# HKUST-Aerial-Robotics/VINS-Mono

Measured on AMD Instinct MI355X. Metric: sliding-window BA solves/sec (Estimator::optimization: 8-iteration dogleg solve + marginalization), higher is better.
Workload: dtype f64; 1 GPU; batch of 256 independent EuRoC-shape windows per step and GPU (K=11 frames, ~150 landmarks, 10 IMU factors, ~600 projection factors, 75-dim marginalization prior, max 8 iterations, MARGIN_OLD marginalization); windows resident in HBM; consecutive steps are issued to 16 HIP streams (independent batches in flight); windows_per_gpu=256, batches_in_flight=16, parallelism=independent batches x1 (no collectives)

## Files before the change

include/vinsgpu.h:

```cpp
#ifndef VINSGPU_H
#define VINSGPU_H
#include <stddef.h>
#include <stdint.h>
#ifdef __cplusplus
extern "C" {
#endif

#define VG_ABI_VERSION 12
#define VG_MAX_ITERS 32

typedef enum {
    VG_OK = 0,
    VG_ERR_BAD_ARG = -1,
    VG_ERR_HIP = -2,
    VG_ERR_UNSUPPORTED = -3,
    VG_ERR_NUMERIC = -4,
    VG_ERR_NO_DEVICE = -5
} vg_status;

typedef struct vg_handle vg_handle;

int vg_abi_version(void);
int vg_create(vg_handle** out);
typedef struct vg_config {
// ... 300 lines not shown
       VG_BA_KERNEL_BIG_SCHUR, VG_BA_KERNEL_BIG_SOLVE, VG_BA_KERNEL_BIG_STEP, VG_BA_KERNEL_COUNT };
int vg_ba_batch_run_profiled(vg_handle* h, float* ms, int* n);
int vg_ba_batch_flops_by_kernel(vg_handle* h, double* flops);
int vg_ba_batch_info(vg_handle* h, double* flops_per_run, double* bytes_in, double* bytes_out, int* lds_bytes);
int vg_ba_batch_flops(vg_handle* h, double* solve_flops, double* marg_flops);

typedef int (*vg_allreduce_fn)(void* user, double* device_buf, size_t count, void* stream);
int vg_ba_set_allreduce(vg_handle* h, vg_allreduce_fn fn, void* user);
int vg_ba_set_large_window(vg_handle* h, int force);

#define VG_RCCL_ID_BYTES 128
int vg_rccl_unique_id(char* id128);
int vg_ba_rccl_init(vg_handle* h, int nranks, int rank, const char* id128);
int vg_ba_rccl_finalize(vg_handle* h);

enum { VG_LAUNCH_DIRECT = 0, VG_LAUNCH_GRAPH = 1 };
#ifndef VG_LAUNCH_DEFAULT
#define VG_LAUNCH_DEFAULT VG_LAUNCH_DIRECT
#endif
int vg_ba_set_launch_mode(vg_handle* h, int mode);
int vg_ba_launch_stats(vg_handle* h, int* mode, long long* graph_launches, long long* graph_captures);
int vg_ba_set_fused_min_windows(vg_handle* h, int min_windows);
int vg_ba_batch_is_fused(vg_handle* h);

int vg_ba_reserve(vg_handle* h, int max_landmarks, int max_factors, int max_obs, int max_prior_n);

typedef struct {
    int n_features;
    const int* feature_id;
    const int* start_frame;
    const int* n_obs;
    const int* solve_flag;
    const double* depth;
    const double* obs;
} vg_ba_tracks;

typedef struct {
    int max_features;
    int max_new_obs;
    int max_landmarks;
    int max_factors;
    double init_depth;
    double min_parallax;
} vg_ba_seq_config;

typedef struct {
// ... 446 lines not shown
```

vins-mono_amd/ba.py:

```python
import time
import ctypes as C
import numpy as np

from . import lib

VG_MAX_ITERS = 32
VG_MARGIN_OLD, VG_MARGIN_SECOND_NEW, VG_MARGIN_NONE = 0, 1, 2
VG_MARG_SQRT, VG_MARG_EIGEN = 0, 1
MARGPATH_STAGE1 = (None, 'direct', 'block_lds', 'block_glb', 'vh_eig', 'jacobi_lds', 'jacobi_glb') + (None,) * 9
MARGPATH_CERT = (None, 'passed', 'failed', None)
MARGPATH_SCHUR = (None, 'lds', 'glb', None)
MARGPATH_STAGE2 = (None, 'sqrt', 'sqrt_glb', 'vh_eig', 'jacobi_lds', 'jacobi_glb') + (None,) * 10
VG_IMU_INFO_FACTOR, VG_IMU_INFO_REFERENCE = 0, 1
VG_OK = 0
VG_ABI_VERSION = 12
VG_LAUNCH_DIRECT, VG_LAUNCH_GRAPH = 0, 1
VG_LAUNCH_DEFAULT = VG_LAUNCH_DIRECT
VG_PRIOR_RESIDENT = -1
_pd = C.POINTER(C.c_double)
_pi = C.POINTER(C.c_int)


class ImuPreint(C.Structure):
    _fields_ = [("sum_dt", C.c_double), ("delta_p", C.c_double * 3), ("delta_q", C.c_double * 4),
                ("delta_v", C.c_double * 3), ("linearized_ba", C.c_double * 3), ("linearized_bg", C.c_double * 3),
                ("jacobian", C.c_double * 225), ("covariance", C.c_double * 225), ("valid", C.c_int), ("_pad", C.c_int)]


class Problem(C.Structure):
    _fields_ = [("K", C.c_int), ("L", C.c_int), ("n_obs", C.c_int),
                ("pose", _pd), ("speedbias", _pd), ("ex_pose", _pd), ("td", C.c_double), ("inv_depth", _pd),
# ... 292 lines not shown
        L.vg_create.argtypes = [C.POINTER(C.c_void_p)]
        L.vg_destroy.argtypes = [C.c_void_p]
        L.vg_sync.argtypes = [C.c_void_p]
        L.vg_last_error.argtypes = [C.c_void_p]
        L.vg_last_error.restype = C.c_char_p
        L.vg_timer_start.argtypes = [C.c_void_p]
        L.vg_timer_stop.argtypes = [C.c_void_p, C.POINTER(C.c_float)]
        L.vg_ba_batch_upload.argtypes = [C.c_void_p, C.c_int, C.POINTER(C.POINTER(Problem)), _pi]
        L.vg_ba_batch_run_async.argtypes = [C.c_void_p]
        L.vg_ba_batch_download.argtypes = [C.c_void_p, C.c_int, C.POINTER(C.POINTER(State)), C.POINTER(Summary),
                                           C.POINTER(C.POINTER(Prior))]
        L.vg_ba_batch_download_state.argtypes = [C.c_void_p, C.c_int, C.POINTER(C.POINTER(State)), C.POINTER(Summary)]
        L.vg_ba_batch_download_prior.argtypes = [C.c_void_p, C.c_int, C.POINTER(C.POINTER(Prior))]
        L.vg_ba_batch_run_timed.argtypes = [C.c_void_p, C.POINTER(C.c_float), C.POINTER(C.c_float)]
        L.vg_ba_batch_run_profiled.argtypes = [C.c_void_p, C.POINTER(C.c_float), _pi]
        L.vg_ba_batch_flops_by_kernel.argtypes = [C.c_void_p, _pd]
        L.vg_ba_batch_info.argtypes = [C.c_void_p, _pd, _pd, _pd, _pi]
        L.vg_ba_batch_flops.argtypes = [C.c_void_p, _pd, _pd]
        L.vg_ba_eval_factors.argtypes = [C.c_void_p, C.POINTER(Problem), _pd, _pd, _pd, _pd, _pd]
        L.vg_ba_set_large_window.argtypes = [C.c_void_p, C.c_int]
        L.vg_ba_set_marg_mode.argtypes = [C.c_void_p, C.c_int]
        L.vg_ba_set_launch_mode.argtypes = [C.c_void_p, C.c_int]
        L.vg_ba_set_fused_min_windows.argtypes = [C.c_void_p, C.c_int]
        L.vg_host_register.argtypes = [C.c_void_p, C.c_void_p, C.c_size_t]
        L.vg_host_unregister.argtypes = [C.c_void_p, C.c_void_p]
        L.vg_ba_launch_stats.argtypes = [C.c_void_p, _pi, C.POINTER(C.c_longlong), C.POINTER(C.c_longlong)]
        if hasattr(L, 'vg_ba_rccl_init'):
            L.vg_ba_rccl_init.argtypes = [C.c_void_p, C.c_int, C.c_int, C.c_char_p]
            L.vg_ba_rccl_finalize.argtypes = [C.c_void_p]
        L.vg_ba_set_allreduce.argtypes = [C.c_void_p, ALLREDUCE_FN, C.c_void_p]
        L.vg_ba_reduce_layout.argtypes = [C.c_void_p, C.POINTER(C.c_size_t), C.POINTER(C.c_size_t)]
        L.vg_triangulate.argtypes = [C.c_void_p, C.c_int, _pd, _pd, _pd, _pd, C.c_int, _pi, _pi, _pi, _pd, C.c_double, _pd]
        L.vg_imu_preintegrate.argtypes = [C.c_void_p, C.c_int, _pi, _pd, _pd, _pd, _pd, C.POINTER(ImuPreint)]
        L.vg_ba_reserve.argtypes = [C.c_void_p, C.c_int, C.c_int, C.c_int, C.c_int]
        L.vg_ba_seq_begin.argtypes = [C.c_void_p, C.c_int, C.POINTER(SeqConfig), C.POINTER(C.POINTER(Problem)), C.POINTER(C.POINTER(Tracks))]
        L.vg_ba_seq_step_async.argtypes = [C.c_void_p, C.c_int, C.POINTER(C.POINTER(Frame))]
        L.vg_ba_seq_info.argtypes = [C.c_void_p, C.c_int, _pi]
        L.vg_ba_seq_get_tracks.argtypes = [C.c_void_p, C.c_int, C.c_int, _pi, _pi, _pi, _pi, _pi, _pd, _pd]
        L.vg_ba_seq_end.argtypes = [C.c_void_p]
        L.vg_ba_seq_export.argtypes = [C.c_void_p, C.c_int, _pd, _pd, _pd, _pd, C.POINTER(ImuPreint), C.POINTER(Prior)]
        L.vg_ba_seq_import.argtypes = [C.c_void_p, C.c_int, C.POINTER(Problem), C.POINTER(Tracks)]
        if hasattr(L, "vg_ba_seq_imu_begin"):
            L.vg_ba_seq_imu_begin.argtypes = [C.c_void_p, C.c_int, C.POINTER(SeqImuConfig), _pd]
            L.vg_ba_seq_step_imu_async.argtypes = [C.c_void_p, C.c_int, C.POINTER(C.POINTER(FrameImu))]
            L.vg_ba_seq_imu_get.argtypes = [C.c_void_p, C.c_int, _pd, _pd, _pd]
            L.vg_ba_seq_imu_set.argtypes = [C.c_void_p, C.c_int, _pd]
# ... 70 lines not shown
            n = len(self._packed)
            arr = (C.POINTER(Problem) * n)(*[C.pointer(p.struct) for p in self._packed])
        mf = np.ascontiguousarray(margin_flags if margin_flags is not None else [VG_MARGIN_NONE] * n, dtype=np.int32)
        self._margin = mf
        t0 = time.perf_counter()
        self._chk(self.lib.vg_ba_batch_upload(self.h, n, arr, _ip(mf)), "vg_ba_batch_upload")
        self.last_upload_call_ms = (time.perf_counter() - t0) * 1e3

    def ba_run_async(self):
        self._chk(self.lib.vg_ba_batch_run_async(self.h), "vg_ba_batch_run_async")

    def ba_set_launch_mode(self, mode):
        self._chk(self.lib.vg_ba_set_launch_mode(self.h, int(mode)), "vg_ba_set_launch_mode")

    def host_register(self, arr):
        self._chk(self.lib.vg_host_register(self.h, C.c_void_p(arr.ctypes.data), C.c_size_t(arr.nbytes)), "vg_host_register")

    def host_unregister(self, arr):
        self._chk(self.lib.vg_host_unregister(self.h, C.c_void_p(arr.ctypes.data)), "vg_host_unregister")

    def ba_set_fused_min_windows(self, n):
        self._chk(self.lib.vg_ba_set_fused_min_windows(self.h, int(n)), "vg_ba_set_fused_min_windows")

    def probe_clocks(self):
        out = (C.c_double * 4)()
        self.lib.vg_probe_clocks.argtypes = [C.c_void_p, C.POINTER(C.c_double)]
        self._chk(self.lib.vg_probe_clocks(self.h, out), "vg_probe_clocks")
        return {"lone_wave": {"ns_per_dependent_fma": out[0], "clock64_ticks_per_us": out[1]},
                "all_cus_loaded": {"ns_per_dependent_fma": out[2], "clock64_ticks_per_us": out[3]}}

    def ba_launch_stats(self):
        mode, nl, ncap = C.c_int(), C.c_longlong(), C.c_longlong()
        self._chk(self.lib.vg_ba_launch_stats(self.h, C.byref(mode), C.byref(nl), C.byref(ncap)), "vg_ba_launch_stats")
        return {"mode": "graph" if mode.value == VG_LAUNCH_GRAPH else "direct", "graph_launches": nl.value, "graph_captures": ncap.value}

    def ba_set_marg_mode(self, mode):
        self._chk(self.lib.vg_ba_set_marg_mode(self.h, int(mode)), "vg_ba_set_marg_mode")

    def ba_marg_info(self, window=0):
        self.lib.vg_ba_batch_marg_info.argtypes = [C.c_void_p, C.c_int, C.POINTER(C.c_int)]
        out = (C.c_int * 8)()
        self._chk(self.lib.vg_ba_batch_marg_info(self.h, int(window), out), "vg_ba_batch_marg_info")
        w = int(out[6])
        return dict(valid=int(out[0]), n=int(out[1]), m=int(out[2]), nblocks=int(out[3]), eig1=int(out[4]), eig2=int(out[5]), word=w,
                    stage1=MARGPATH_STAGE1[w & 0xf], cert=MARGPATH_CERT[(w >> 4) & 3], schur=MARGPATH_SCHUR[(w >> 6) & 3],
                    stage2=MARGPATH_STAGE2[(w >> 8) & 0xf])
# ... 584 lines not shown
```

vins-mono_amd/csrc/ba_carve.h:

```cpp
#pragma once

#ifdef __HIPCC__
#define BA_HD __host__ __device__ inline
#else
#define BA_HD inline
#endif
BA_HD int ba_up(int v, int m) { return (v + m - 1) / m * m; }
BA_HD int ba_max(int a, int b) { return a > b ? a : b; }
BA_HD int ba_min(int a, int b) { return a < b ? a : b; }

#define BA_CU_LDS (160 * 1024)
#define BA_LDS_STATIC (8192 + 512)
#define BA_LDS_MAX_LINACC (159 * 1024)
#define BA_LDS_MAX_LIN (128 * 1024)

#define IMU_U 225
#define IMU_PANEL 480
#define PRO_WS 256
#define PRO_WS_REF 512
#define MG_REC 42
#define MG_PRV_PAD 480
#define BA_NST(K, Kp) ba_up(7 * (Kp) + 9 * (K) + 8, 2)

struct LinLds { int U, panels, dx, part, end, need_imu, need_prior; };
BA_HD LinLds lin_lds(int nb, int Ncap) {
    LinLds c;
    c.U = 0; c.panels = ba_up(nb * IMU_U, 2);
    c.dx = 0; c.part = Ncap;
    c.need_imu = c.panels + nb * IMU_PANEL; c.need_prior = c.part + 4 * Ncap;
    c.end = ba_max(c.need_imu, c.need_prior);
    return c;
}

#define LA_NT BA_NT
#define LA_RS 33
#define LA_NPW 6
#define LA_MAXP 13
#define LA_QCAP 80
#define LA_PAIR 90
#define LA_NCH 64
#define LA_MAXCHF 512
static_assert(LA_QCAP <= 128, "the pair prefix of ba_linacc_proj_kernel takes two pairs per lane of one wavefront");
struct LinaccLds {
    int rec, P, key, x, end;
    int i_lstart, i_posx, i_pstart, i_wcnt, i_end;
    int need_imu, need_prior;
};
#define LA_FIXED_INTS (LA_NCH + LA_QCAP + 2 + LA_NT / 64 * LA_QCAP)
BA_HD int linacc_chf(int K, int Kp) {
    const int avail = (BA_CU_LDS - BA_LDS_STATIC) / 8, per = LA_RS + 1;
    const int chf = (avail - BA_NST(K, Kp) - Kp * (Kp - 1) / 2 * LA_PAIR - per - LA_FIXED_INTS / 2) / per;
    return ba_min(chf & ~1, LA_MAXCHF);
// ... 75 lines not shown
```

vins-mono_amd/csrc/ba_host.hip:

```cpp
#include "vg_range.h"
#include <hip/hip_runtime.h>
#include <algorithm>
#include <chrono>
#include <cmath>
#include <cstdio>
#include <cstdlib>
#include <cstring>
#include <string>
#include <thread>
#include <vector>
#include "ba_layout_fn.h"
#include "vg_handle.h"
#include "../../include/vinsgpu.h"

struct BaFork { hipStream_t aux; hipEvent_t fork, join; };
extern "C" hipError_t ba_launch_solve(const BaLayout& L, const BaLayout* dL, const BaPtrs& P, int rounds, hipStream_t stream,
                                      hipEvent_t* ev, int* kinds, int* n_launches, const BaFork* fk);
typedef int (*BaAllReduce)(void* user, double* buf, size_t count, void* stream);
extern "C" hipError_t ba_launch_solve_big(const BaLayout& L, const BaLayout* dL, const BaPtrs& P, int rounds, int slack, hipStream_t stream,
                                          BaAllReduce allreduce, void* user, int* hook_rc, hipEvent_t* ev, int* kinds, int* n_launches);
extern "C" hipError_t ba_launch_eval_factors(const BaLayout& L, const BaLayout* dL, const BaPtrs& P, double* proj_r, double* proj_J,
                                            double* imu_r, double* imu_J, double* prior_r, hipStream_t stream);
extern "C" const char* ba_failed_launch();
extern "C" hipError_t ba_prepare_launch();
extern "C" hipError_t ba_launch_marg(const BaLayout& L, const BaLayout* dL, const BaPtrs& P, hipStream_t stream);
extern "C" hipError_t ba_launch_carry_prior(int nwin, const double* mout, const int* miout, int mo_J0, int mo_r0, int mo_x0, int mo_stride,
                                            int mi_stride, int mcap, int x0cap, double* pri, int po_x0, int po_r0, int po_J0, int pld,
                                            int pstride, hipStream_t stream);

#define HIPCHK(h, expr)                                                                            \
    do {                                                                                           \
        hipError_t _e = (expr);                                                                    \
        if (_e != hipSuccess) {                                                                    \
            (h)->err = std::string(#expr) + ": " + hipGetErrorString(_e);                          \
            return VG_ERR_HIP;                                                                     \
        }                                                                                          \
    } while (0)

static inline int up(int v, int m) { return (v + m - 1) / m * m; }

// ... 533 lines not shown
    B.solved_recorded = false; B.marg_info_ready = false;
    B.uploaded = true;
    return VG_OK;
}

static void note_marg_run(BaBatch& B) {
    B.mout_pending = true;
    B.run_margin = B.margin;
    B.run_nwin = B.nwin; B.run_K = B.L.K;
    B.run_mo_J0 = B.L.mo_J0; B.run_mo_r0 = B.L.mo_r0; B.run_mo_x0 = B.L.mo_x0; B.run_mo_stride = B.L.mo_stride;
    B.run_mi_stride = B.L.mi_stride; B.run_mcap = B.L.mcap;
}

#define BA_BIG_SLACK 8
static int launch_solve(vg_handle* h, hipEvent_t* ev = nullptr, int* kinds = nullptr, int* n_launches = nullptr) {
    BaBatch& B = h->ba;
    hipError_t e;
    if (B.L.big) {
        int hook_rc = 0;
        e = ba_launch_solve_big(B.L, B.dL, B.P, B.rounds + BA_BIG_SLACK, BA_BIG_SLACK, h->stream, (BaAllReduce)B.allreduce, B.allreduce_user, &hook_rc,
                                ev, kinds, n_launches);
        if (e != hipSuccess && hook_rc) { h->err = "all-reduce hook returned " + std::to_string(hook_rc); return VG_ERR_HIP; }
    } else {
        e = ba_launch_solve(B.L, B.dL, B.P, B.rounds, h->stream, ev, kinds, n_launches, nullptr);
    }
    if (e != hipSuccess) { h->err = std::string("launch of ") + ba_failed_launch() + ": " + hipGetErrorString(e); return VG_ERR_HIP; }
    return VG_OK;
}

static int resolve_launch_mode(BaBatch& B) {
    if (B.launch_mode < 0) {
        const char* e = B.no_env ? nullptr : getenv("VG_BA_LAUNCH_MODE");
        B.launch_mode = VG_LAUNCH_DEFAULT;
        if (e && !strcmp(e, "graph")) B.launch_mode = VG_LAUNCH_GRAPH;
        if (e && !strcmp(e, "direct")) B.launch_mode = VG_LAUNCH_DIRECT;
    }
    return B.launch_mode;
}
static void graph_key(const BaBatch& B, BaBatch::GraphKey& k) {
    const BaLayout& L = B.L;
    k.dL = B.dL; k.P = B.P;
    const int d[12] = {L.nwin, L.nig, L.nprw, L.nbf, L.nba, L.lds_pro, L.lds_lin, L.lds_solve, B.rounds, L.la_on, L.lds_linacc, L.big};
    memcpy(k.dims, d, sizeof(d));
}
static void graph_drop(BaBatch& B) {
    if (B.gexec) (void)hipGraphExecDestroy(B.gexec);
    B.gexec = nullptr;
}
extern "C" void ba_graph_release(vg_handle* h) { graph_drop(h->ba); }
static int launch_solve_graph(vg_handle* h) {
    BaBatch& B = h->ba;
    BaBatch::GraphKey k;
    graph_key(B, k);
    if (!B.gexec || memcmp(&k, &B.gkey, sizeof(k)) != 0) {
        graph_drop(B);
        HIPCHK(h, ba_prepare_launch());
        if (hipStreamBeginCapture(h->stream, hipStreamCaptureModeThreadLocal) != hipSuccess) {
            (void)hipGetLastError();
            B.graph_unavailable = true;
            return launch_solve(h);
        }
        const int rc = launch_solve(h);
        hipGraph_t g = nullptr;
        const hipError_t ec = hipStreamEndCapture(h->stream, &g);
        if (rc) { if (g) (void)hipGraphDestroy(g); return rc; }
// ... 5 lines not shown
        ++B.n_graph_captures;
    }
    HIPCHK(h, hipGraphLaunch(B.gexec, h->stream));
    ++B.n_graph_launches;
    return VG_OK;
}
static int launch_solve_in_mode(vg_handle* h) {
    BaBatch& B = h->ba;
    const bool graph = resolve_launch_mode(B) == VG_LAUNCH_GRAPH && !B.L.big && !B.graph_unavailable;
    return graph ? launch_solve_graph(h) : launch_solve(h);
}
extern "C" int vg_ba_set_launch_mode(vg_handle* h, int mode) {
    if (!h || (mode != VG_LAUNCH_DIRECT && mode != VG_LAUNCH_GRAPH)) return VG_ERR_BAD_ARG;
    h->ba.launch_mode = mode;
    if (mode == VG_LAUNCH_DIRECT) graph_drop(h->ba);
    return VG_OK;
}
extern "C" int vg_ba_set_fused_min_windows(vg_handle* h, int min_windows) {
    if (!h || min_windows < 0) return VG_ERR_BAD_ARG;
    h->ba.fused_min = min_windows;
    h->ba.uploaded = false;
    return VG_OK;
}
extern "C" int vg_ba_batch_is_fused(vg_handle* h) {
    if (!h || !h->ba.uploaded) return VG_ERR_BAD_ARG;
    return h->ba.L.la_on ? 1 : 0;
}
extern "C" int vg_ba_batch_marg_info(vg_handle* h, int window, int out[8]) {
    if (!h || !out || !h->ba.uploaded || window < 0 || window >= h->ba.nwin) return VG_ERR_BAD_ARG;
    BaBatch& B = h->ba;
    if (!B.marg_info_ready) { h->err = "vg_ba_batch_marg_info before the priors of this run were downloaded"; return VG_ERR_BAD_ARG; }
    const int* mi = B.h_miout.data() + (size_t)window * B.L.mi_stride;
    for (int k = 0; k < 8; ++k) out[k] = mi[k];
    return VG_OK;
}
extern "C" int vg_ba_launch_stats(vg_handle* h, int* mode, long long* graph_launches, long long* graph_captures) {
    if (!h) return VG_ERR_BAD_ARG;
    if (mode) *mode = h->ba.graph_unavailable ? VG_LAUNCH_DIRECT : resolve_launch_mode(h->ba);
    if (graph_launches) *graph_launches = h->ba.n_graph_launches;
    if (graph_captures) *graph_captures = h->ba.n_graph_captures;
    return VG_OK;
}

extern "C" int vg_ba_batch_run_async(vg_handle* h) {
    VG_RANGE("vg_ba_batch_run_async");
    if (!h || !h->ba.uploaded) return VG_ERR_BAD_ARG;
// ... 82 lines not shown
    }
    HIPCHK(h, hipEventSynchronize(ev[nl]));
    for (int k = 0; k < VG_BA_KERNEL_COUNT; ++k) { ms[k] = 0.f; n[k] = 0; }
    for (int i = 0; i < nl; ++i) {
        float t = 0.f;
        HIPCHK(h, hipEventElapsedTime(&t, ev[i], ev[i + 1]));
        ms[kinds[i] & 0xff] += t;
        if (!(kinds[i] & 0x100)) n[kinds[i] & 0xff] += 1;
    }
    for (int i = 0; i < nev; ++i) (void)hipEventDestroy(ev[i]);
    return VG_OK;
}

extern "C" int vg_ba_batch_flops(vg_handle* h, double* solve_flops, double* marg_flops) {
    if (!h || !h->ba.uploaded) return VG_ERR_BAD_ARG;
    if (solve_flops) *solve_flops = h->ba.flops - h->ba.flops_marg;
    if (marg_flops) *marg_flops = h->ba.flops_marg;
    return VG_OK;
}

extern "C" int vg_ba_batch_flops_by_kernel(vg_handle* h, double* flops) {
    if (!h || !h->ba.uploaded || !flops) return VG_ERR_BAD_ARG;
    for (int k = 0; k < VG_BA_KERNEL_COUNT; ++k) flops[k] = h->ba.flops_k[k];
    return VG_OK;
}

extern "C" int vg_ba_batch_info(vg_handle* h, double* flops, double* bytes_in, double* bytes_out, int* lds_bytes) {
    if (!h || !h->ba.uploaded) return VG_ERR_BAD_ARG;
    if (flops) *flops = h->ba.flops;
    if (bytes_in) *bytes_in = h->ba.bytes_in;
    if (bytes_out) *bytes_out = h->ba.bytes_out;
    if (lds_bytes) *lds_bytes = h->ba.L.lds_solve;
    return VG_OK;
}

static int unpack_states(vg_handle* h, int nwin, vg_ba_state* const* st, vg_ba_summary* sum) {
    BaBatch& B = h->ba;
    const BaLayout& L = B.L;
    std::vector<int> worst_t(64, VG_OK);
    tl_pack_cap = h->ba.pack_threads;
    for_windows(nwin, [&](int t, int w) {
        int& worst = worst_t[t];
        const double* o = B.h_out.data() + (size_t)w * L.ostride;
        const int* io = B.h_iout.data() + (size_t)w * L.oi_stride;
        if (st && st[w]) {
            vg_ba_state* s = st[w];
// ... 1055 lines not shown
```

vins-mono_amd/csrc/ba_pipeline.hip:

```cpp
#include <hip/hip_runtime.h>
#include <vector>
#include <mutex>
#include <cstring>
#include <cstdlib>
#include "ba_layout.h"
#include "ba_factors.h"
#include "../../include/vinsgpu.h"

extern __shared__ __attribute__((aligned(16))) char bp_smem[];

#ifdef BA_SOLVE_W8_TU
#undef BA_PROFILE_DETAIL
#undef BA_DEBUG_DUMP
namespace vg_w8 {
#endif

#define NOINL __device__ __noinline__
#define AS_LDS(p) ((lds_d*)(p))
#define AS_LDS_C(p) ((const lds_d*)(p))
#define AS_GLB(p) ((glb_d*)(p))
#define AS_GLB_C(p) ((const glb_d*)(p))
#define AS_GLB_CI(p) ((const glb_i*)(p))
template <bool BIG> struct MovT { typedef lds_d D; typedef lds_i I; };
template <> struct MovT<true> { typedef glb_d D; typedef glb_i I; };
// ... 349 lines not shown
        if (c.tid == 7) x[7 * L.Kp + 9 * L.K + 7] = c.di[L.do_td];
        for (int k = c.tid; k < c.nL; k += BA_NT) c.sc[L.so_lam + k] = c.di[L.do_lam + k];
        if (c.tid < C_NCTL) {
            double v = 0.0;
            if (c.tid == C_RADIUS) v = 1e4;
            if (c.tid == C_MU || c.tid == C_MUSOLVED) v = 1e-8;
            if (c.tid == C_T0) v = (double)wall_clock64();
            c.sc[L.so_ctl + c.tid] = v;
        }
    }
    DP_ADD(40);
    if (all || (part >= 1 && part <= nI)) {
        const int fbeg = all ? 0 : (part - 1) * BA_NW, fend = all ? L.K - 1 : part * BA_NW;
        if (L.imu_info) imu_sqrt_info_ref(c, fbeg, fend);
        else imu_sqrt_info(c, fbeg, fend);
    }
    DP_ADD(41);
    if (c.nprior && (all || part > nI)) {
        const bool do_copy = all || part == nI + 1, do_prod = all || part == nI + 2;
        const int n = c.nprior;
        const double* J0 = c.pri + L.po_J0;
        double* Hp = c.sc + L.so_Hp;
        if (do_copy) {
            double* J0t = c.sc + L.so_J0t;
            for (int wk = c.tid; wk < n * n; wk += BA_NT) { const int r = wk / n, cc = wk % n; J0t[cc * L.Ncap + r] = J0[r * L.pld + cc]; }
        }
        __syncthreads();
        DP_ADD(42);
        if (!do_prod) {
        } else if ((size_t)n * n * 8 <= (size_t)L.lds_pro) {
            double* J0s = LDSB;
            for (int wk = c.tid; wk < n * n; wk += BA_NT) J0s[wk] = J0[(wk / n) * L.pld + wk % n];
            __syncthreads();
            DP_ADD(43);
            const int T = (n + 15) >> 4, ntile = T * (T + 1) / 2, nks = (n + 3) >> 2;
            const int wave = c.tid >> 6, lane = c.tid & 63, li = lane & 15, lk = lane >> 4;
            for (int t = wave; t < ntile; t += BA_NT / 64) {
                int ta, tb;
                tri_decode(t, ta, tb);
                const int ca = 16 * ta + li, cb = 16 * tb + li;
                double4_t acc = (double4_t){0, 0, 0, 0};
                for (int ks = 0; ks < nks; ++ks) {
                    const int r = 4 * ks + lk;
                    const double av = (r < n && ca < n) ? J0s[r * n + ca] : 0.0;
                    const double bv = (r < n && cb < n) ? J0s[r * n + cb] : 0.0;
                    acc = __builtin_amdgcn_mfma_f64_16x16x4f64(av, bv, acc, 0, 0, 0);
                }
#pragma unroll
// ... 3511 lines not shown
        exc[7] = L.t ? exx[7] + vU[col_td(L)] : exx[7];
    }
    for (int k = c.tid; k < nL; k += BA_NT) lamc[k] = lam[k] + sl[k] * ((c_gt * gtl[k] + c_gn * gnl[k]) / dgl[k]);
    __syncthreads();
    {
        double sd = 0.0;
        const int nx = 7 * L.Kp + 9 * L.K + (L.e ? 7 : 0);
        for (int k = c.tid; k < nx; k += BA_NT) { const double d = x[k] - xc[k]; sd += d * d; }
        if (L.t && c.tid == 0) { const double d = x[7 * L.Kp + 9 * L.K + 7] - xc[7 * L.Kp + 9 * L.K + 7]; sd += d * d; }
        double sn = state_sqnorm_share(L, xc, nullptr, 0, c.tid, BA_NT);
        block_sum2(red, BA_NW, c.lane, c.wave, sd, sn);
        s.step2c = sd;
        s.xn2c = sn;
    }
    if (c.tid == 0) {
        out[L.oo_trace + 2 * VG_MAX_ITERS + slot] = model_change;
        out[L.oo_trace + 4 * VG_MAX_ITERS + slot] = s.dnorm;
    }
    s.pending = 1;
    __syncthreads();
    if (c.tid == 0) ctl_store(s, ctlp);
}

extern "C" __global__ __launch_bounds__(256) void ba_final_kernel(const BaLayout* __restrict__ Lp, BaPtrs P) {
    const BaLayout& L = *Lp;
    Ctx c;
    const int w = blockIdx.x;
    ctx_init(c, Lp, P, w);
    const int NT = 256;
    double* ctlp = c.sc + L.so_ctl;
    double* out = P.out + (size_t)w * L.ostride;
    int* iout = P.iout + (size_t)w * L.oi_stride;
    Ctl s;
    ctl_load(s, ctlp);
    if (s.pending) {
        double cs;
        if (L.big) {
            const double* scal = P.rb1 + (size_t)w * L.rb1_len + L.rb1_scal;
            cs = scal[RB1_COST] + sum_partials(c.sc + L.so_part + L.nbf, L.nig + L.nprw);
            s.step_norm = sqrt(s.step2c + scal[RB1_STEP2]);
            s.x_norm_c = sqrt(s.xn2c + scal[RB1_LAM2]);
        } else {
            cs = sum_partials(c.sc + L.so_part, L.nbl);
        }
        const bool acc = judge_candidate(s, cs, L, out, iout, c.tid);
        if (acc && !(s.cost == s.cost)) { s.status = VG_ERR_NUMERIC; s.term = VG_TERM_FAILURE; }
    }
    const double* x = c.sc + L.so_x + s.cur * L.nst;
    const double* lam = c.sc + L.so_lam + s.cur * L.Lcap;
    const double* p0_in = c.di + L.do_pose;
    double Rs0[9], R00[9], y0[3], y00[3], rot[9];
    q_to_R(p0_in + 3, Rs0);
    q_to_R(x + 3, R00);
    R2ypr_dev(Rs0, y0);
    R2ypr_dev(R00, y00);
    const double yd = (y0[0] - y00[0]) / 180.0 * M_PI;
    rot[0] = cos(yd); rot[1] = -sin(yd); rot[2] = 0;
    rot[3] = sin(yd); rot[4] = cos(yd);  rot[5] = 0;
    rot[6] = 0;       rot[7] = 0;        rot[8] = 1;
    if (fabs(fabs(y0[1]) - 90) < 1.0 || fabs(fabs(y00[1]) - 90) < 1.0) m3_mul_t(Rs0, R00, rot);
    for (int i = c.tid; i < L.Kp; i += NT) {
        double q[4] = {x[7 * i + 3], x[7 * i + 4], x[7 * i + 5], x[7 * i + 6]};
        q_normalize(q);
        double Rq[9], Ri[9], qo[4], d[3], po[3];
        q_to_R(q, Rq);
        m3_mul(rot, Rq, Ri);
        R_to_q(Ri, qo);
        d[0] = x[7 * i] - x[0]; d[1] = x[7 * i + 1] - x[1]; d[2] = x[7 * i + 2] - x[2];
        m3_vec(rot, d, po);
        double* o = out + L.oo_pose + 7 * i;
        o[0] = po[0] + p0_in[0]; o[1] = po[1] + p0_in[1]; o[2] = po[2] + p0_in[2];
        o[3] = qo[0]; o[4] = qo[1]; o[5] = qo[2]; o[6] = qo[3];
        if (i < L.K) {
            const double* sb = x + 7 * L.Kp + 9 * i;
            double vo[3];
            m3_vec(rot, sb, vo);
            double* os = out + L.oo_sb + 9 * i;
            os[0] = vo[0]; os[1] = vo[1]; os[2] = vo[2];
            for (int k = 3; k < 9; ++k) os[k] = sb[k];
        }
    }
    if (c.tid == 0) {
        const double* exx = x + 7 * L.Kp + 9 * L.K;
        double Rcm[9], qo[4];
        q_to_R(exx + 3, Rcm);
        R_to_q(Rcm, qo);
        double* o = out + L.oo_ex;
        o[0] = exx[0]; o[1] = exx[1]; o[2] = exx[2]; o[3] = qo[0]; o[4] = qo[1]; o[5] = qo[2]; o[6] = qo[3];
        out[L.oo_td] = exx[7];
        out[L.oo_sum + 0] = s.init_cost;
        out[L.oo_sum + 1] = s.cost;
        out[L.oo_sum + 2] = s.radius;
        for (int k = 0; k < 9; ++k) out[L.oo_sum + 3 + k] = rot[k];
        for (int k = 0; k < 3; ++k) out[L.oo_sum + 12 + k] = x[k];
        iout[0] = s.status; iout[1] = s.term; iout[2] = s.it; iout[3] = s.nacc;
        s.done = 1;
        ctl_store(s, ctlp);
    }
    for (int k = c.tid; k < c.nL; k += NT) out[L.oo_lam + k] = 1.0 / (1.0 / lam[k]);
}

extern "C" __global__ __launch_bounds__(BA_NT) void ba_eval_factors_kernel(const BaLayout* __restrict__ Lp, BaPtrs P, double* proj_r,
                                                                       double* proj_J, double* imu_r, double* imu_J, double* prior_r) {
    const BaLayout& L = *Lp;
    Ctx c;
    ctx_init(c, Lp, P, 0);
    const double* x = c.sc + L.so_x;
    const double* lam = c.sc + L.so_lam;
    double* buf = lin_buf(c, 0);
    prior_pass(c, x, buf + L.bo_pr, nullptr, LDSB);
    __syncthreads();
    const int nimu = L.K - 1;
    for (int w = c.tid; w < nimu * 31; w += BA_NT) {
        const int f = w / 31, col = w % 31;
        if (!c.ia[L.io_imu_valid + f]) continue;
        const double* pre = c.di + L.do_imu + f * BA_IMU_STRIDE;
        const double* U = c.sc + L.so_imuU + f * IMU_U;
        ImuCtx ic;
        imu_ctx<true>(pre, st_pose(L, x, f), st_sb(L, x, f), st_pose(L, x, f + 1), st_sb(L, x, f + 1), c.gnorm, ic);
        double raw[15];
        if (col < 30) imu_raw_col(ic, pre, col, raw);
        else { for (int q = 0; q < 15; ++q) raw[q] = ic.r[q]; }
// ... 39 lines not shown
    if (e == hipSuccess) e = hipFuncSetAttribute((const void*)ba_solve_big_tail_kernel, hipFuncAttributeMaxDynamicSharedMemorySize, BA_CU_LDS);
    if (e == hipSuccess) e = hipFuncSetAttribute((const void*)ba_prologue_kernel, hipFuncAttributeMaxDynamicSharedMemorySize, BA_CU_LDS);
    if (e == hipSuccess) e = hipFuncSetAttribute((const void*)ba_linacc_proj_kernel, hipFuncAttributeMaxDynamicSharedMemorySize, BA_LDS_MAX_LINACC);
    if (e == hipSuccess) e = hipFuncSetAttribute((const void*)ba_linearize_imu_kernel, hipFuncAttributeMaxDynamicSharedMemorySize, BA_LDS_MAX_LIN);
    if (e == hipSuccess) e = hipFuncSetAttribute((const void*)ba_eval_factors_kernel, hipFuncAttributeMaxDynamicSharedMemorySize, BA_LDS_MAX_LIN);
    if (e == hipSuccess && dev >= 0 && dev < 64) done_mask |= 1ull << dev;
    return e;
}

extern "C" hipError_t ba_prepare_launch() { return set_lds_attrs(); }

static const char* g_failed_launch = "";
extern "C" const char* ba_failed_launch() { return g_failed_launch; }
#define LAUNCH(name, grid, block, lds, ...)                                              \
    do {                                                                                 \
        hipLaunchKernelGGL(name, grid, block, lds, stream, __VA_ARGS__);                 \
        const hipError_t _le = hipGetLastError();                                        \
        if (_le != hipSuccess) { g_failed_launch = #name; return _le; }                  \
        if (ev) { const hipError_t _ee = hipEventRecord(ev[nev++], stream); if (_ee != hipSuccess) return _ee; } \
    } while (0)

struct BaFork { hipStream_t aux; hipEvent_t fork, join; };
extern "C" hipError_t ba_launch_solve(const BaLayout& L, const BaLayout* dL, const BaPtrs& P, int rounds, hipStream_t stream,
                                      hipEvent_t* ev, int* kinds, int* n_launches, const BaFork* fk) {
    hipError_t e = set_lds_attrs();
    if (e != hipSuccess) { g_failed_launch = "hipFuncSetAttribute"; return e; }
    int nev = 0;
    if (ev) { e = hipEventRecord(ev[nev++], stream); if (e != hipSuccess) return e; }
    const bool forked = fk && fk->aux && !ev && !L.la_on;
    int nk = 0;
    LAUNCH(ba_prologue_kernel, dim3(L.nwin, pro_grid_y(L.pro_split, L.K)), dim3(BA_NT), L.lds_pro, dL, P);
    if (kinds) kinds[nk++] = 0;
    for (int r = 0; r <= rounds; ++r) {
        const int cost_only = r == rounds ? 1 : 0;
        const bool fused = L.la_on && !cost_only;
        if (fused) {
        } else if (forked) {
            if ((e = hipEventRecord(fk->fork, stream)) != hipSuccess) return e;
            if ((e = hipStreamWaitEvent(fk->aux, fk->fork, 0)) != hipSuccess) return e;
            hipLaunchKernelGGL(ba_linearize_imu_kernel, dim3(L.nig + L.nprw, L.nwin), dim3(BA_NT), L.lds_lin, fk->aux, dL, P, cost_only);
            if ((e = hipGetLastError()) != hipSuccess) { g_failed_launch = "ba_linearize_imu_kernel"; return e; }
            if ((e = hipEventRecord(fk->join, fk->aux)) != hipSuccess) return e;
        } else {
            LAUNCH(ba_linearize_imu_kernel, dim3(L.nig + L.nprw, L.nwin), dim3(BA_NT), L.lds_lin, dL, P, cost_only);
        }
        if (fused) LAUNCH(ba_linacc_proj_kernel, dim3(L.nwin), dim3(LA_NT), L.lds_linacc, dL, P);
        else LAUNCH(ba_linearize_proj_kernel, dim3(L.nbf, L.nwin), dim3(BA_LIN_NT), 0, dL, P, cost_only);
        if (kinds) { if (!forked && !fused) kinds[nk++] = 1; kinds[nk++] = fused ? 2 : 1; }
        if (r == rounds) {
            if (forked && (e = hipStreamWaitEvent(stream, fk->join, 0)) != hipSuccess) return e;
            break;
        }
        if (!fused) LAUNCH(ba_accumulate_kernel, dim3(L.nba * ((L.nwin + 7) / 8) * 8), dim3(BA_ACC_NT), 0, dL, P);
        if (forked && (e = hipStreamWaitEvent(stream, fk->join, 0)) != hipSuccess) return e;
        if (L.sv_w8) LAUNCH(ba_solve_w8_kernel, dim3(L.nwin), dim3(2 * SV_NT), L.lds_solve_w8, dL, P);
        else LAUNCH(ba_solve_kernel, dim3(L.nwin), dim3(SV_NT), L.lds_solve, dL, P);
        if (kinds) { if (!fused) kinds[nk++] = 2; kinds[nk++] = 3; }
    }
    LAUNCH(ba_final_kernel, dim3(L.nwin), dim3(256), 0, dL, P);
    if (kinds) kinds[nk++] = 4;
    if (n_launches) *n_launches = nk;
    return hipSuccess;
}

typedef int (*BaAllReduce)(void* user, double* buf, size_t count, void* stream);
extern "C" hipError_t ba_launch_solve_big(const BaLayout& L, const BaLayout* dL, const BaPtrs& P, int rounds, int slack, hipStream_t stream,
                                          BaAllReduce allreduce, void* user, int* hook_rc, hipEvent_t* ev, int* kinds, int* n_launches) {
    hipError_t e = set_lds_attrs();
    if (e != hipSuccess) { g_failed_launch = "hipFuncSetAttribute"; return e; }
    int nev = 0, nk = 0;
    if (ev) { e = hipEventRecord(ev[nev++], stream); if (e != hipSuccess) return e; }
    if (hook_rc) *hook_rc = 0;
    const size_t n1 = (size_t)L.nwin * L.rb1_len, n2 = (size_t)L.nwin * RB2_LEN;
#define REDUCE(buf, n)                                                                   \
    do {                                                                                 \
        if (allreduce) {                                                                 \
            const int _rc = allreduce(user, buf, n, (void*)stream);                      \
            if (_rc) { if (hook_rc) *hook_rc = _rc; g_failed_launch = "all-reduce hook"; return hipErrorInvalidValue; } \
        }                                                                                \
    } while (0)
#define KIND(k) do { if (kinds) kinds[nk++] = (k); } while (0)
    LAUNCH(ba_prologue_kernel, dim3(L.nwin, pro_grid_y(L.pro_split, L.K)), dim3(BA_NT), L.lds_pro, dL, P); KIND(0);
// ... 46 lines not shown
```

vins-mono_amd/csrc/vg_handle.h:

```cpp
#pragma once
#include <hip/hip_runtime.h>
#include <string>
#include <vector>
#include "ba_layout.h"

template <typename T>
struct PinnedBuf {
    T* p = nullptr;
    size_t cap = 0, n = 0;
    hipError_t resize(size_t need) {
        n = need;
        if (need <= cap) return hipSuccess;
        if (p) (void)hipHostFree(p);
        p = nullptr; cap = 0;
        hipError_t e = hipHostMalloc((void**)&p, need * sizeof(T), hipHostMallocDefault);
        if (e == hipSuccess) cap = need;
        return e;
    }
    T* data() { return p; }
    size_t size() const { return n; }
    void release() { if (p) (void)hipHostFree(p); p = nullptr; cap = n = 0; }
};

struct SeqDev {
// ... 58 lines not shown
    BaLayout* dL = nullptr;
    size_t dL_bytes = 0;
    BaLayout dL_host;
    bool dL_valid = false;
    BaPtrs P = {nullptr, nullptr, nullptr, nullptr, nullptr, nullptr, nullptr, nullptr, nullptr, nullptr, nullptr};
    size_t cap_ia = 0, cap_di = 0, cap_sc = 0, cap_out = 0, cap_iout = 0, cap_mout = 0, cap_miout = 0, cap_mscr = 0, cap_rb1 = 0, cap_rb2 = 0;
    std::vector<int> margin, nL;
    PinnedBuf<int> h_iout, h_miout;
    PinnedBuf<double> h_out, h_mout;
    int* h_ia = nullptr;
    double* h_di = nullptr;
    size_t hcap_ia = 0, hcap_di = 0;
    int nwin = 0;
    int rounds = 0;
    bool uploaded = false, any_margin = false;
    bool solved_recorded = false;
    bool marg_info_ready = false;
    bool force_large = false;
    int marg_mode = 0;
    int imu_info_mode = 0;
    int res_L = 0, res_F = 0, res_O = 0, res_N = 0;
    bool res_relo = false;
    int fused_min = -1;
    bool no_env = false;
    int pack_threads = 0;
    BaSeq seq;
    void* allreduce = nullptr;
    void* allreduce_user = nullptr;
    struct PriorSlot { int n = 0, nb = 0; std::vector<int> kind, idx; };
    std::vector<PriorSlot> slot;
    int slot_K = 0, slot_po_r0 = 0, slot_pld = 0, slot_pstride = 0;
    size_t cap_pri = 0;
    double* h_pri = nullptr;
    size_t hcap_pri = 0;
    bool mout_pending = false;
    std::vector<int> run_margin;
    int run_nwin = 0, run_K = 0, run_mo_J0 = 0, run_mo_r0 = 0, run_mo_x0 = 0, run_mo_stride = 0, run_mi_stride = 0, run_mcap = 0;
    struct GraphKey {
        const void* dL = nullptr;
        BaPtrs P = {nullptr, nullptr, nullptr, nullptr, nullptr, nullptr, nullptr, nullptr, nullptr, nullptr, nullptr};
        int dims[12] = {0, 0, 0, 0, 0, 0, 0, 0, 0, 0, 0, 0};
    };
    int launch_mode = -1;
    hipGraphExec_t gexec = nullptr;
    GraphKey gkey;
    bool graph_unavailable = false;
    long long n_graph_launches = 0, n_graph_captures = 0;
    double flops = 0, flops_marg = 0, bytes_in = 0, bytes_out = 0;
    double flops_k[12] = {0, 0, 0, 0, 0, 0, 0, 0, 0, 0, 0, 0};
};

struct FeState;

struct vg_handle {
    int device = 0;
    hipStream_t stream = nullptr;
    hipEvent_t ev0 = nullptr, ev1 = nullptr, ev2 = nullptr;
    hipStream_t aux = nullptr;
    hipEvent_t ev_fork = nullptr, ev_join = nullptr;
    std::string err;
    BaBatch ba;
    FeState* fe = nullptr;
    void* rccl_comm = nullptr;
    void* imu_buf = nullptr;
// ... 10 lines not shown
```

Measured before the change: 185,300 solves/s.

## Add optional fused tail kernel merging final cost evaluation into final kernel

Adds an opt-in tail mode where, in the fused-linearization path, the last cost-only round is skipped and the candidate cost is computed inside a new final kernel variant, removing one kernel launch per solve. It also unrolls the prior Jacobian transpose copy to issue eight loads before their stores, for more memory-level parallelism. The tail mode defaults to the old separate-launch path, so by default only the copy change runs. The fused tail uses more LDS and threads in the final kernel.

```diff
diff --git a/include/vinsgpu.h b/include/vinsgpu.h
--- a/include/vinsgpu.h
+++ b/include/vinsgpu.h
@@ -346,6 +346,9 @@
 int vg_ba_launch_stats(vg_handle* h, int* mode, long long* graph_launches, long long* graph_captures);
 int vg_ba_set_fused_min_windows(vg_handle* h, int min_windows);
 int vg_ba_batch_is_fused(vg_handle* h);
+#define VG_BA_TAIL_FUSED 0
+#define VG_BA_TAIL_LAUNCHES 1
+int vg_ba_set_tail_mode(vg_handle* h, int mode);
 
 int vg_ba_reserve(vg_handle* h, int max_landmarks, int max_factors, int max_obs, int max_prior_n);
 
diff --git a/vins-mono_amd/ba.py b/vins-mono_amd/ba.py
--- a/vins-mono_amd/ba.py
+++ b/vins-mono_amd/ba.py
@@ -7,6 +7,7 @@
 VG_MAX_ITERS = 32
 VG_MARGIN_OLD, VG_MARGIN_SECOND_NEW, VG_MARGIN_NONE = 0, 1, 2
 VG_MARG_SQRT, VG_MARG_EIGEN = 0, 1
+VG_BA_TAIL_FUSED, VG_BA_TAIL_LAUNCHES = 0, 1
 MARGPATH_STAGE1 = (None, 'direct', 'block_lds', 'block_glb', 'vh_eig', 'jacobi_lds', 'jacobi_glb') + (None,) * 9
 MARGPATH_CERT = (None, 'passed', 'failed', None)
 MARGPATH_SCHUR = (None, 'lds', 'glb', None)
@@ -345,6 +346,8 @@
         L.vg_ba_set_marg_mode.argtypes = [C.c_void_p, C.c_int]
         L.vg_ba_set_launch_mode.argtypes = [C.c_void_p, C.c_int]
         L.vg_ba_set_fused_min_windows.argtypes = [C.c_void_p, C.c_int]
+        if hasattr(L, "vg_ba_set_tail_mode"):
+            L.vg_ba_set_tail_mode.argtypes = [C.c_void_p, C.c_int]
         L.vg_host_register.argtypes = [C.c_void_p, C.c_void_p, C.c_size_t]
         L.vg_host_unregister.argtypes = [C.c_void_p, C.c_void_p]
         L.vg_ba_launch_stats.argtypes = [C.c_void_p, _pi, C.POINTER(C.c_longlong), C.POINTER(C.c_longlong)]
@@ -461,6 +464,9 @@
     def ba_set_fused_min_windows(self, n):
         self._chk(self.lib.vg_ba_set_fused_min_windows(self.h, int(n)), "vg_ba_set_fused_min_windows")
 
+    def ba_set_tail_mode(self, mode):
+        self._chk(self.lib.vg_ba_set_tail_mode(self.h, int(mode)), "vg_ba_set_tail_mode")
+
     def probe_clocks(self):
         out = (C.c_double * 4)()
         self.lib.vg_probe_clocks.argtypes = [C.c_void_p, C.POINTER(C.c_double)]
diff --git a/vins-mono_amd/csrc/ba_carve.h b/vins-mono_amd/csrc/ba_carve.h
--- a/vins-mono_amd/csrc/ba_carve.h
+++ b/vins-mono_amd/csrc/ba_carve.h
@@ -28,6 +28,15 @@
     c.U = 0; c.panels = ba_up(nb * IMU_U, 2);
     c.dx = 0; c.part = Ncap;
     c.need_imu = c.panels + nb * IMU_PANEL; c.need_prior = c.part + 4 * Ncap;
+    c.end = ba_max(c.need_imu, c.need_prior);
+    return c;
+}
+
+struct TailLds { int need_imu, need_prior, end; };
+BA_HD TailLds tail_lds(int nb, int Ncap) {
+    const LinLds l = lin_lds(nb, Ncap);
+    TailLds c;
+    c.need_imu = l.panels; c.need_prior = l.need_prior;
     c.end = ba_max(c.need_imu, c.need_prior);
     return c;
 }
diff --git a/vins-mono_amd/csrc/ba_host.hip b/vins-mono_amd/csrc/ba_host.hip
--- a/vins-mono_amd/csrc/ba_host.hip
+++ b/vins-mono_amd/csrc/ba_host.hip
@@ -15,7 +15,7 @@
 
 struct BaFork { hipStream_t aux; hipEvent_t fork, join; };
 extern "C" hipError_t ba_launch_solve(const BaLayout& L, const BaLayout* dL, const BaPtrs& P, int rounds, hipStream_t stream,
-                                      hipEvent_t* ev, int* kinds, int* n_launches, const BaFork* fk);
+                                      hipEvent_t* ev, int* kinds, int* n_launches, const BaFork* fk, int tail_mode);
 typedef int (*BaAllReduce)(void* user, double* buf, size_t count, void* stream);
 extern "C" hipError_t ba_launch_solve_big(const BaLayout& L, const BaLayout* dL, const BaPtrs& P, int rounds, int slack, hipStream_t stream,
                                           BaAllReduce allreduce, void* user, int* hook_rc, hipEvent_t* ev, int* kinds, int* n_launches);
@@ -595,7 +595,7 @@
                                 ev, kinds, n_launches);
         if (e != hipSuccess && hook_rc) { h->err = "all-reduce hook returned " + std::to_string(hook_rc); return VG_ERR_HIP; }
     } else {
-        e = ba_launch_solve(B.L, B.dL, B.P, B.rounds, h->stream, ev, kinds, n_launches, nullptr);
+        e = ba_launch_solve(B.L, B.dL, B.P, B.rounds, h->stream, ev, kinds, n_launches, nullptr, B.tail_mode);
     }
     if (e != hipSuccess) { h->err = std::string("launch of ") + ba_failed_launch() + ": " + hipGetErrorString(e); return VG_ERR_HIP; }
     return VG_OK;
@@ -613,7 +613,7 @@
 static void graph_key(const BaBatch& B, BaBatch::GraphKey& k) {
     const BaLayout& L = B.L;
     k.dL = B.dL; k.P = B.P;
-    const int d[12] = {L.nwin, L.nig, L.nprw, L.nbf, L.nba, L.lds_pro, L.lds_lin, L.lds_solve, B.rounds, L.la_on, L.lds_linacc, L.big};
+    const int d[14] = {L.nwin, L.nig, L.nprw, L.nbf, L.nba, L.lds_pro, L.lds_lin, L.lds_solve, B.rounds, L.la_on, L.lds_linacc, L.big, B.tail_mode, 0};
     memcpy(k.dims, d, sizeof(d));
 }
 static void graph_drop(BaBatch& B) {
@@ -665,6 +665,11 @@
     h->ba.uploaded = false;
     return VG_OK;
 }
+extern "C" int vg_ba_set_tail_mode(vg_handle* h, int mode) {
+    if (!h || (mode != 0 && mode != 1)) return VG_ERR_BAD_ARG;
+    h->ba.tail_mode = mode;
+    return VG_OK;
+}
 extern "C" int vg_ba_batch_is_fused(vg_handle* h) {
     if (!h || !h->ba.uploaded) return VG_ERR_BAD_ARG;
     return h->ba.L.la_on ? 1 : 0;
@@ -793,6 +798,7 @@
 extern "C" int vg_ba_batch_flops_by_kernel(vg_handle* h, double* flops) {
     if (!h || !h->ba.uploaded || !flops) return VG_ERR_BAD_ARG;
     for (int k = 0; k < VG_BA_KERNEL_COUNT; ++k) flops[k] = h->ba.flops_k[k];
+    if (h->ba.L.la_on && h->ba.tail_mode == 0) { flops[VG_BA_KERNEL_FINAL] += flops[VG_BA_KERNEL_LINEARIZE]; flops[VG_BA_KERNEL_LINEARIZE] = 0.0; }
     return VG_OK;
 }
 
diff --git a/vins-mono_amd/csrc/ba_pipeline.hip b/vins-mono_amd/csrc/ba_pipeline.hip
--- a/vins-mono_amd/csrc/ba_pipeline.hip
+++ b/vins-mono_amd/csrc/ba_pipeline.hip
@@ -395,8 +395,16 @@
         const double* J0 = c.pri + L.po_J0;
         double* Hp = c.sc + L.so_Hp;
         if (do_copy) {
-            double* J0t = c.sc + L.so_J0t;
-            for (int wk = c.tid; wk < n * n; wk += BA_NT) { const int r = wk / n, cc = wk % n; J0t[cc * L.Ncap + r] = J0[r * L.pld + cc]; }
+            glb_d* J0t = AS_GLB(c.sc + L.so_J0t);
+            const glb_d* J0g = AS_GLB_C(J0);
+            const int nn = n * n;
+            for (int w0 = c.tid; w0 < nn; w0 += 8 * BA_NT) {
+                double jv[8];
+#pragma unroll
+                for (int u = 0; u < 8; ++u) { const int wk = w0 + u * BA_NT, r = wk / n, cc = wk - r * n; jv[u] = wk < nn ? J0g[r * L.pld + cc] : 0.0; }
+#pragma unroll
+                for (int u = 0; u < 8; ++u) { const int wk = w0 + u * BA_NT, r = wk / n, cc = wk - r * n; if (wk < nn) J0t[cc * L.Ncap + r] = jv[u]; }
+            }
         }
         __syncthreads();
         DP_ADD(42);
@@ -3954,12 +3962,51 @@
     if (c.tid == 0) ctl_store(s, ctlp);
 }
 
-extern "C" __global__ __launch_bounds__(256) void ba_final_kernel(const BaLayout* __restrict__ Lp, BaPtrs P) {
+NOINL double tail_cost(const Ctx& c_in, int cand, double* red) {
+    const Ctx c = c_in;
+    const BaLayout L = *c.Lp;
+    const double* x = c.sc + L.so_x + cand * L.nst;
+    const double* lam = c.sc + L.so_lam + cand * L.Lcap;
+    double* buf = lin_buf(c, cand);
+    glb_d* part = AS_GLB(c.sc + L.so_part);
+    const int WPT = BA_LIN_NT / 64, TPT = BA_NT / BA_LIN_NT;
+    double cs = 0.0;
+    for (int b0 = 0; b0 < L.nbf; b0 += TPT) {
+        const int f = b0 * BA_LIN_NT + c.tid;
+        double share = 0.0;
+        if (f < c.nF) share = proj_cost(c, f, x, lam);
+        share = wave_sum_all(share);
+        __syncthreads();
+        if (c.lane == 0) red[c.wave] = share;
+        __syncthreads();
+        for (int t = 0; t < TPT && b0 + t < L.nbf; ++t) {
+            double tot = 0.0;
+            for (int w = 0; w < WPT; ++w) tot += red[t * WPT + w];
+            tot = uni(tot);
+            if (c.tid == 0) part[b0 + t] = tot;
+            cs += tot;
+        }
+    }
+    for (int g = 0; g < L.nig + L.nprw; ++g) {
+        double share = 0.0;
+        if (g < L.nig) {
+            const int fbeg = g * L.igs, fend = (fbeg + L.igs < L.K - 1) ? fbeg + L.igs : L.K - 1;
+            share = imu_pass<false>(c, x, buf + L.bo_imuJ, fbeg, fend);
+        }
+        if (L.nprw ? g == L.nig : g == 0) share += prior_pass(c, x, buf + L.bo_pr, nullptr, LDSB);
+        const double tot = block_sum(red, BA_NW, c.lane, c.wave, share);
+        if (c.tid == 0) part[L.nbf + g] = tot;
+        cs += tot;
+    }
+    return uni(cs);
+}
+
+template <int NT, bool TAIL>
+__device__ __forceinline__ void final_body(const BaLayout* __restrict__ Lp, const BaPtrs& P, double* red) {
     const BaLayout& L = *Lp;
     Ctx c;
     const int w = blockIdx.x;
     ctx_init(c, Lp, P, w);
-    const int NT = 256;
     double* ctlp = c.sc + L.so_ctl;
     double* out = P.out + (size_t)w * L.ostride;
     int* iout = P.iout + (size_t)w * L.oi_stride;
@@ -3967,7 +4014,9 @@
     ctl_load(s, ctlp);
     if (s.pending) {
         double cs;
-        if (L.big) {
+        if (TAIL && !s.done) {
+            cs = tail_cost(c, s.cur ^ 1, red);
+        } else if (L.big) {
             const double* scal = P.rb1 + (size_t)w * L.rb1_len + L.rb1_scal;
             cs = scal[RB1_COST] + sum_partials(c.sc + L.so_part + L.nbf, L.nig + L.nprw);
             s.step_norm = sqrt(s.step2c + scal[RB1_STEP2]);
@@ -3978,6 +4027,8 @@
         const bool acc = judge_candidate(s, cs, L, out, iout, c.tid);
         if (acc && !(s.cost == s.cost)) { s.status = VG_ERR_NUMERIC; s.term = VG_TERM_FAILURE; }
     }
+    constexpr int NG = TAIL ? 128 : NT;
+    if (TAIL && c.tid >= NG) return;
     const double* x = c.sc + L.so_x + s.cur * L.nst;
     const double* lam = c.sc + L.so_lam + s.cur * L.Lcap;
     const double* p0_in = c.di + L.do_pose;
@@ -3991,7 +4042,7 @@
     rot[3] = sin(yd); rot[4] = cos(yd);  rot[5] = 0;
     rot[6] = 0;       rot[7] = 0;        rot[8] = 1;
     if (fabs(fabs(y0[1]) - 90) < 1.0 || fabs(fabs(y00[1]) - 90) < 1.0) m3_mul_t(Rs0, R00, rot);
-    for (int i = c.tid; i < L.Kp; i += NT) {
+    for (int i = c.tid; i < L.Kp; i += NG) {
         double q[4] = {x[7 * i + 3], x[7 * i + 4], x[7 * i + 5], x[7 * i + 6]};
         q_normalize(q);
         double Rq[9], Ri[9], qo[4], d[3], po[3];
@@ -4029,7 +4080,12 @@
         s.done = 1;
         ctl_store(s, ctlp);
     }
-    for (int k = c.tid; k < c.nL; k += NT) out[L.oo_lam + k] = 1.0 / (1.0 / lam[k]);
+    for (int k = c.tid; k < c.nL; k += NG) out[L.oo_lam + k] = 1.0 / (1.0 / lam[k]);
+}
+extern "C" __global__ __launch_bounds__(256) void ba_final_kernel(const BaLayout* __restrict__ Lp, BaPtrs P) { final_body<256, false>(Lp, P, nullptr); }
+extern "C" __global__ __launch_bounds__(BA_NT) void ba_final_tail_kernel(const BaLayout* __restrict__ Lp, BaPtrs P) {
+    __shared__ double red[2 * BA_NW];
+    final_body<BA_NT, true>(Lp, P, red);
 }
 
 extern "C" __global__ __launch_bounds__(BA_NT) void ba_eval_factors_kernel(const BaLayout* __restrict__ Lp, BaPtrs P, double* proj_r,
@@ -4115,17 +4171,19 @@
 
 struct BaFork { hipStream_t aux; hipEvent_t fork, join; };
 extern "C" hipError_t ba_launch_solve(const BaLayout& L, const BaLayout* dL, const BaPtrs& P, int rounds, hipStream_t stream,
-                                      hipEvent_t* ev, int* kinds, int* n_launches, const BaFork* fk) {
+                                      hipEvent_t* ev, int* kinds, int* n_launches, const BaFork* fk, int tail_mode) {
     hipError_t e = set_lds_attrs();
     if (e != hipSuccess) { g_failed_launch = "hipFuncSetAttribute"; return e; }
     int nev = 0;
     if (ev) { e = hipEventRecord(ev[nev++], stream); if (e != hipSuccess) return e; }
     const bool forked = fk && fk->aux && !ev && !L.la_on;
+    const bool fused_tail = L.la_on && tail_mode == 0;
     int nk = 0;
     LAUNCH(ba_prologue_kernel, dim3(L.nwin, pro_grid_y(L.pro_split, L.K)), dim3(BA_NT), L.lds_pro, dL, P);
     if (kinds) kinds[nk++] = 0;
     for (int r = 0; r <= rounds; ++r) {
         const int cost_only = r == rounds ? 1 : 0;
+        if (cost_only && fused_tail) break;
         const bool fused = L.la_on && !cost_only;
         if (fused) {
         } else if (forked) {
@@ -4150,7 +4208,12 @@
         else LAUNCH(ba_solve_kernel, dim3(L.nwin), dim3(SV_NT), L.lds_solve, dL, P);
         if (kinds) { if (!fused) kinds[nk++] = 2; kinds[nk++] = 3; }
     }
-    LAUNCH(ba_final_kernel, dim3(L.nwin), dim3(256), 0, dL, P);
+    if (fused_tail) {
+        const int lds = 8 * tail_lds(ba_min(ba_min(L.K - 1, BA_IMU_BATCH), L.igs), L.Ncap).end;
+        LAUNCH(ba_final_tail_kernel, dim3(L.nwin), dim3(BA_NT), lds, dL, P);
+    } else {
+        LAUNCH(ba_final_kernel, dim3(L.nwin), dim3(256), 0, dL, P);
+    }
     if (kinds) kinds[nk++] = 4;
     if (n_launches) *n_launches = nk;
     return hipSuccess;
diff --git a/vins-mono_amd/csrc/vg_handle.h b/vins-mono_amd/csrc/vg_handle.h
--- a/vins-mono_amd/csrc/vg_handle.h
+++ b/vins-mono_amd/csrc/vg_handle.h
@@ -104,6 +104,7 @@
     int res_L = 0, res_F = 0, res_O = 0, res_N = 0;
     bool res_relo = false;
     int fused_min = -1;
+    int tail_mode = 1;
     bool no_env = false;
     int pack_threads = 0;
     BaSeq seq;
@@ -121,7 +122,7 @@
     struct GraphKey {
         const void* dL = nullptr;
         BaPtrs P = {nullptr, nullptr, nullptr, nullptr, nullptr, nullptr, nullptr, nullptr, nullptr, nullptr, nullptr};
-        int dims[12] = {0, 0, 0, 0, 0, 0, 0, 0, 0, 0, 0, 0};
+        int dims[14] = {0, 0, 0, 0, 0, 0, 0, 0, 0, 0, 0, 0, 0, 0};
     };
     int launch_mode = -1;
     hipGraphExec_t gexec = nullptr;
```

Result: faster. 187,200 solves/s (median of 6 runs) (+1.0%).
